# zoltanmaric/h264-fer

Hardware: AMD Instinct MI355X
Metric: macroblocks/sec encode (1080p full-search ME) + bit-exact bitstream vs ref (higher is better)
Workload: dtype u8; 1 GPU; 1080p IPPP encode, full-search +-16 ME (BASELINE configs[2]); content=textured, coded_size=1920x1072, streams_per_gpu=256, contexts_per_gpu=1, gop=30, qp=12, window=32, maxdiff=3, parallelism=1 x 256 independent closed-GOP streams

## Files before the change

h264-fer_amd/csrc/fer_api.hip:

```cpp
#include "fer_ctx.h"
#include "fer_pic_host.h"
#include <stdlib.h>
#include <string.h>

static const int k_qpc[52] = {0,  1,  2,  3,  4,  5,  6,  7,  8,  9,  10, 11, 12, 13, 14, 15, 16, 17,
                              18, 19, 20, 21, 22, 23, 24, 25, 26, 27, 28, 29, 29, 30, 31, 32, 32, 33,
                              34, 34, 35, 35, 36, 36, 37, 37, 37, 38, 38, 38, 39, 39, 39, 39};

extern "C" int ferhip_chroma_qp(int qpy) { return k_qpc[qpy < 0 ? 0 : (qpy > 51 ? 51 : qpy)]; }

int PinnedRing::create(size_t bytes_per_slot, size_t second_bytes)
{
    slot_bytes = bytes_per_slot + second_bytes;
    second_off = bytes_per_slot;
    if (!mem) CK(hipHostMalloc((void **)&mem, slot_bytes * FER_HDR_SLOTS));
    for (int i = 0; i < FER_HDR_SLOTS; i++)
        if (!ev[i]) CK(hipEventCreateWithFlags(&ev[i], hipEventDisableTiming));
    return 0;
}
void *PinnedRing::next()
{
    slot = (slot + 1) % FER_HDR_SLOTS;
    if (hipEventSynchronize(ev[slot]) != hipSuccess) return nullptr;
    return mem + (size_t)slot * slot_bytes;
// ... 1074 lines not shown
    {
        ProfScope ps(c, FERHIP_PH_ME_PRE, 1);
        fer_launch_me_pre(c->d, c->st);
    }
    {
        ProfScope ps(c, FERHIP_PH_ME_WALK, 1);
        fer_launch_me_walk(c->d, c->st);
    }
    if (c->d.speculate) {
        ProfScope ps(c, FERHIP_PH_ME_SPEC, 1);
        fer_launch_me_spec(c->d, c->st);
    }
    {
        ProfScope ps(c, FERHIP_PH_ME_RESOLVE, 1);
        c->d.serial = c->d.serial % 0x7ffffff0 + 1;
        fer_launch_me_resolve(c->d, c->st);
    }
    fer_launch_basic_stat(c->d, c->st);
    fer_launch_p_resid(c->d, c->st);
    CK(hipStreamSynchronize(c->st));
    CK(hipGetLastError());
    return 0;
}

extern "C" size_t ferhip_read_buffer(ferhip_ctx *c, int which, void *dst, size_t cap)
{
    if (!c || !dst) return 0;
    (void)hipSetDevice(c->device);
    if (ctx_sync(c) != hipSuccess) return 0;
    FerDev &d = c->d;
    size_t nm = (size_t)d.nmb * d.S;
    const void *src = nullptr;
    size_t n = 0;
    switch (which) {
    case FERHIP_BUF_INTERP: {
        n = d.ysz * 16 * d.S;
        if (n > cap) return 0;
        for (int pl = 0; pl < 16 * d.S; pl++)
            if (hipMemcpy2D((uint8_t *)dst + (size_t)pl * d.ysz, (size_t)d.W, d.interp + (size_t)pl * d.iplane + d.ioff, (size_t)d.ipitch,
                            (size_t)d.W, (size_t)d.H, hipMemcpyDeviceToHost) != hipSuccess)
                return 0;
        return n;
    }
    case FERHIP_BUF_FEAT: {
        n = d.ysz * 96 * d.S * 2;
        if (n > cap) return 0;
        if (dalloc(c, &d.feat, d.ysz * 96 * d.S)) return 0;
        if (hipDeviceSynchronize() != hipSuccess) return 0;
        fer_launch_features(d, c->st);
        src = d.feat;
        break;
    }
    case FERHIP_BUF_SORTPOS: src = d.sort_pos; n = d.ysz * d.S * 4; break;
    case FERHIP_BUF_KOLIKO: {
        n = (size_t)16385 * d.S * 4;
        if (n > cap) return 0;
        if (hipStreamSynchronize(c->st) != hipSuccess) return 0;
        for (int s = 0; s < d.S; s++) {
            int *o = (int *)dst + (size_t)s * 16385;
            if (hipMemcpy2D(o, 4, d.kol2 + (size_t)s * 16384 * d.kt, (size_t)d.kt * 4, 4, 16385, hipMemcpyDeviceToHost) != hipSuccess)
                return 0;
            for (int a = 0; a <= 16384; a++) o[a] -= (int)((size_t)s * d.ysz);
        }
        return n;
    }
    case FERHIP_BUF_MBTYPE: src = d.mb_type; n = nm * 4; break;
    case FERHIP_BUF_MV: src = d.mv; n = nm * 16; break;
    case FERHIP_BUF_MVD: src = d.mvd; n = nm * 16; break;
    case FERHIP_BUF_LEVELS: src = d.levels; n = nm * FER_LEVELS * 2; break;
    case FERHIP_BUF_CBP: src = d.cbp; n = nm * 2; break;
    case FERHIP_BUF_TC: src = d.tc; n = nm * 24; break;
    case FERHIP_BUF_I4MODE: src = d.i4mode; n = nm * 16; break;
    case FERHIP_BUF_TIMING: src = d.timing; n = 64 * 8; break;
    case FERHIP_BUF_ST2N: src = d.st2n; n = nm * 16; break;
    case FERHIP_BUF_SUMA: src = d.suma; n = nm * 4 * 5 * 4; break;
    case FERHIP_BUF_ST3: src = d.st3; n = nm * 4 * 33 * 3 * 4; break;
    case FERHIP_BUF_ST3N: src = d.st3n; n = nm * 16; break;
    case FERHIP_BUF_V0: src = d.v0; n = nm * 16; break;
    case FERHIP_BUF_SPEC_HDR: src = d.spec_hdr; n = nm * 4 * 16; break;
    case FERHIP_BUF_SPEC_L1: src = d.spec_l1; n = nm * 4 * 17 * 8; break;
    case FERHIP_BUF_SPEC_L2: src = d.spec_l2; n = nm * 4 * 33 * 8; break;
    case FERHIP_BUF_ST2: src = d.st2; n = nm * 4 * FER_ST2_CAP * 8; break;
    case FERHIP_BUF_SPEC_STAT: src = d.spec_stat; n = 8 * 8; break;
    case FERHIP_BUF_MBSIZE: src = d.mbsize; n = nm * 8; break;
    case FERHIP_BUF_CUR:
    case FERHIP_BUF_REF: {
        n = d.ysz * 3 / 2 * d.S;
        if (n > cap) return 0;
        uint8_t *set = c->planes[which == FERHIP_BUF_CUR ? c->cur_set : c->cur_set ^ 1];
        if (copy_frames(c, set, nullptr, (uint8_t *)dst, hipMemcpyDeviceToHost)) return 0;
        if (hipStreamSynchronize(c->st) != hipSuccess) return 0;
        return n;
    }
    default: return 0;
    }
    if (n > cap) return 0;
    if (hipStreamSynchronize(c->st) != hipSuccess) return 0;
    if (hipMemcpy(dst, src, n, hipMemcpyDeviceToHost) != hipSuccess) return 0;
    return n;
}
```

h264-fer_amd/csrc/fer_internal.h:

```cpp
#pragma once
#include "fer_dev.h"
#include "../../include/ferhip.h"

struct FerSortTmp {
    uint4 *rec1;
    uint16_t *keyT;
    uint8_t *dig2;
    uint16_t *skey;
    uint32_t *rec_tmp;
    void *tmp;
    size_t tmp_bytes;
};

size_t fer_sort_tmp_bytes(int n, int S);
void fer_launch_refprep(const FerDev &d, FerSortTmp &t, const int *types, hipStream_t st);
void fer_launch_interp(const FerDev &d, hipStream_t st);
void fer_launch_features(const FerDev &d, hipStream_t st);
void fer_launch_sort(const FerDev &d, FerSortTmp &t, hipStream_t st);
void fer_launch_sort_keys(const FerDev &d, FerSortTmp &t, hipStream_t st);
void fer_launch_sort_radix(const FerDev &d, FerSortTmp &t, hipStream_t st);
void fer_launch_sort_finish(const FerDev &d, FerSortTmp &t, hipStream_t st);
void fer_launch_me_walk(const FerDev &d, hipStream_t st);
void fer_launch_frame_sad(const FerDev &d, const uint8_t *skip, hipStream_t st);
void fer_launch_me_pre(const FerDev &d, hipStream_t st);
void fer_launch_me_spec(const FerDev &d, hipStream_t st);
void fer_launch_me_resolve(const FerDev &d, hipStream_t st);
void fer_launch_basic_stat(const FerDev &d, hipStream_t st);
void fer_launch_p_resid(const FerDev &d, hipStream_t st);
void fer_launch_intra(const FerDev &d, hipStream_t st);
void fer_launch_cavlc(const FerDev &d, hipStream_t st);
void fer_launch_rc_plan(const FerDev &d, hipStream_t st);
int fer_quality_groups(const FerDev &d);
void fer_launch_quality(const FerDev &d, int flags, int slot, hipStream_t st);
void fer_launch_carry_ref(const FerDev &d, hipStream_t st);
void fer_launch_reset_stream(const FerDev &d, int s, int qpw, hipStream_t st);
struct DecLuts;
const DecLuts *dec_luts(hipStream_t st);
void fer_launch_decode_parse(const FerDev &d, const DecBatch &B, hipStream_t st);
void fer_launch_decode_recon(const FerDev &dslice, bool anyP, bool anyIntra, hipStream_t st);
void fer_launch_decode_out(const FerDev &d, const uint8_t *set, const int2 *map, int n, uint8_t *dst, hipStream_t st);
void fer_launch_pad_ingest(const FerDev &d, uint8_t *set, const uint8_t *src, int dw, int dh, const uint8_t *present, hipStream_t st);
void fer_launch_pic_ingest(const FerDev &d, uint8_t *set, const ferhip_pic *d_pics, int format, int dw, int dh, hipStream_t st);
void fer_launch_pic_emit(const FerDev &d, const uint8_t *set, const ferhip_pic *d_pics, int format, const int *win, hipStream_t st);
void fer_launch_pic_emit_slots(const FerDev &d, const uint8_t *set, const int2 *map, int n, uint8_t *dst, int format, uint32_t pitch_y,
                               uint32_t pitch_c, size_t slot_bytes, const int *win, hipStream_t st);
void fer_launch_pic_ingest_packed(const FerDev &d, uint8_t *set, const ferhip_pic *d_pics, int format, int csc, int dw, int dh, hipStream_t st);
void fer_launch_pic_emit_packed(const FerDev &d, const uint8_t *set, const ferhip_pic *d_pics, const int2 *map, int n, uint8_t *dst, int format,
                                int csc, uint32_t pitch, size_t slot_bytes, const int *win, hipStream_t st);
```

h264-fer_amd/csrc/fer_refprep.hip:

```cpp
#include <cstring>
#include <string.h>
#include <algorithm>
#include "fer_internal.h"

#ifndef IT_W
#define IT_W 128
#define IT_H 8
#endif
typedef short s16x2_t __attribute__((ext_vector_type(2)));
#define IT_PITCH (IT_W + 8)
__global__ __launch_bounds__(256) void k_interp(FerDev d)
{
    __shared__ __attribute__((aligned(16))) uint8_t tile[IT_H + 5][IT_PITCH];
    const int s = blockIdx.y;
    if (d.hdr[s * 4 + 3] != 0) return;
    const int W = d.W, H = d.H;
    const uint8_t *R = d.refY + (size_t)s * d.ysz;
    uint8_t *P = d.interp + (size_t)s * 16 * d.iplane + d.ioff;
    const int tw = (W + IT_W - 1) / IT_W;
    const int t = (int)xcd_swizzle(blockIdx.x, gridDim.x);
    const int x0 = (t % tw) * IT_W, y0 = (t / tw) * IT_H;
    const int tid = threadIdx.x;
    {
        constexpr int NL = ((IT_H + 5) * (IT_PITCH / 4) + 255) / 256;
// ... 203 lines not shown
    int nzero = 0;
#pragma unroll
    for (int j = 0; j < 16 + 7; j++) {
        const int r = g * 16 + j;
        const uint32_t *w = (const uint32_t *)&tile[r][x & ~3];
        const uint32_t lo = __builtin_amdgcn_alignbyte(w[1], w[0], (uint32_t)sh);
        const uint32_t hi = __builtin_amdgcn_alignbyte(w[2], w[1], (uint32_t)sh);
        const int a4 = (int)__builtin_amdgcn_sad_u8(lo, 0u, 0u);
        h4[j & 7] = a4;
        h8[j & 7] = (int)__builtin_amdgcn_sad_u8(hi, 0u, (uint32_t)a4);
        hc[j & 7] = (int)__builtin_amdgcn_sad_u8(hi & 0xffffu, 0u, __builtin_amdgcn_sad_u8(lo & 0xffffu, 0u, 0u));
        if (j >= 7) {
            const int yo = r - 7;
            int k0 = 0, k2 = 0, k4 = 0;
#pragma unroll
            for (int k = 0; k < 8; k++) {
                k0 += h8[k];
                k2 += h4[k];
                k4 += hc[k];
            }
            const int k1 = h8[(j + 1) & 7] + h8[(j + 2) & 7] + h8[(j + 3) & 7] + h8[(j + 4) & 7];
            const int k3 = h8[(j + 1) & 7] + h8[(j + 2) & 7] + h8[(j + 5) & 7] + h8[(j + 6) & 7];
            const uint32_t a = (uint32_t)k0 | ((uint32_t)k1 << 16), b = (uint32_t)k2 | ((uint32_t)k3 << 16), c = (uint32_t)k4;
            stage[x][yo] = (uint16_t)k0;
            const int gx = x0 + x, gy = y0 + yo;
            if (gx < W && gy < H) {
                uint32_t *o = (uint32_t *)(d.feat0 + ((size_t)s * d.ysz + (size_t)gy * W + gx) * 6);
                o[0] = a;
                o[1] = b;
                o[2] = c;
                nzero += k0 == 0;
            }
        }
    }
    if (__any(nzero)) {
        const int tot = wave_sum(nzero);
        if ((tid & 63) == 0 && tot) atomicAdd(&d.zero_cnt[s], tot);
    }
    __syncthreads();
    for (int i = tid; i < F0_T * F0_T / 2; i += 256) {
        const int cx = i >> 5, cy = (i & 31) * 2;
        const int gx = x0 + cx, gy = y0 + cy;
        if (gx < W && gy < H)
            *(uint32_t *)(keyT + (size_t)s * d.ysz + (size_t)gx * H + gy) = (uint32_t)stage[cx][cy] | ((uint32_t)stage[cx][cy + 1] << 16);
    }
}

#ifndef RS_THREADS
#define RS_THREADS 512
#endif
#ifndef RS_ITEMS
#define RS_ITEMS 8
#endif
#define RS_TILE (RS_THREADS * RS_ITEMS)
#define RS_BITS 7
#define RS_ND (1 << RS_BITS)

__global__ __launch_bounds__(RS_THREADS) void k_rs_hist(FerDev d, const uint16_t *keyT, const uint8_t *dig2, uint32_t *hist, int ntiles,
                                                       int pass)
{
    __shared__ unsigned h[RS_ND];
    const int s = blockIdx.y, tile = blockIdx.x, tid = threadIdx.x;
    if (d.hdr[s * 4 + 3] != 0) return;
    const int n = d.W * d.H;
    const size_t g0 = (size_t)s * n;
    if (tid < RS_ND) h[tid] = 0;
    static_assert(RS_ITEMS == 8, "one 16-byte / 8-byte load per thread");
    const int idx = tile * RS_TILE + tid * RS_ITEMS;
    const bool ok = idx < n;
    unsigned dgs[RS_ITEMS];
    if (pass == 0) {
        const uint4 v = ok ? *(const uint4 *)(keyT + g0 + idx) : make_uint4(0, 0, 0, 0);
        const uint32_t w[4] = {v.x, v.y, v.z, v.w};
#pragma unroll
        for (int i = 0; i < RS_ITEMS; i++) dgs[i] = (w[i >> 1] >> (16 * (i & 1))) & (RS_ND - 1);
    } else {
        const uint2 v = ok ? *(const uint2 *)(dig2 + g0 + idx) : make_uint2(0, 0);
        const uint32_t w[2] = {v.x, v.y};
#pragma unroll
        for (int i = 0; i < RS_ITEMS; i++) dgs[i] = (w[i >> 2] >> (8 * (i & 3))) & 0xffu;
    }
    __syncthreads();
#pragma unroll
    for (int i = 0; i < RS_ITEMS; i++) {
        const unsigned dg = dgs[i];
        const unsigned d0 = (unsigned)__builtin_amdgcn_readfirstlane((int)dg);
        const unsigned long long same = __ballot(ok && dg == d0);
        if (same && (tid & 63) == __ffsll((long long)same) - 1) atomicAdd(&h[d0], (unsigned)__popcll(same));
        if (ok && dg != d0) atomicAdd(&h[dg], 1u);
    }
    __syncthreads();
    if (tid < RS_ND) hist[((size_t)s * RS_ND + tid) * ntiles + tile] = h[tid];
}

#define RSS_WAVES 16
__global__ __launch_bounds__(64 * RSS_WAVES) void k_rs_scan(FerDev d, uint32_t *hist, int ntiles)
{
    __shared__ unsigned wtot[RSS_WAVES];
    const int s = blockIdx.x, tid = threadIdx.x, lane = tid & 63, wv = tid >> 6;
    if (d.hdr[s * 4 + 3] != 0) return;
    uint4 *h4 = (uint4 *)(hist + (size_t)s * RS_ND * ntiles);
    const int n4 = RS_ND * ntiles / 4;
    const int per = (n4 + RSS_WAVES - 1) / RSS_WAVES;
    const int u0 = min(wv * per, n4), u1 = min(u0 + per, n4);
    unsigned sum = 0;
    for (int u = u0 + lane; u < u1; u += 64) {
        const uint4 v = h4[u];
        sum += v.x + v.y + v.z + v.w;
    }
    sum = (unsigned)wave_sum((int)sum);
    if (lane == 0) wtot[wv] = sum;
    __syncthreads();
    unsigned carry = 0;
    for (int w = 0; w < wv; w++) carry += wtot[w];
    for (int ub = u0; ub < u1; ub += 64) {
        const int u = ub + lane;
        const uint4 v = u < u1 ? h4[u] : make_uint4(0, 0, 0, 0);
        const unsigned t = v.x + v.y + v.z + v.w;
        unsigned inc = t;
#pragma unroll
        for (int o = 1; o < 64; o <<= 1) {
            const unsigned x = __shfl_up(inc, o);
            if (lane >= o) inc += x;
        }
        const unsigned ex = carry + inc - t;
        if (u < u1) h4[u] = make_uint4(ex, ex + v.x, ex + v.x + v.y, ex + v.x + v.y + v.z);
        carry += __shfl(inc, 63);
    }
}

#define RS_SEG_PITCH 12
__device__ __forceinline__ void rs_divmod(unsigned v, unsigned dv, float rdv, unsigned &qo, unsigned &rem)
{
    int q = (int)((float)v * rdv);
    int r = (int)v - q * (int)dv;
    if (r < 0) {
        q--;
        r += (int)dv;
    }
    if (r >= (int)dv) {
        q++;
        r -= (int)dv;
    }
    qo = (unsigned)q;
    rem = (unsigned)r;
}

template <int PASS>
__global__ __launch_bounds__(RS_THREADS) void k_rs_scatter(FerDev d, const uint8_t *dig2_in, const uint4 *rec_in, uint4 *rec1_out,
                                                          uint8_t *dig2_out, uint32_t *rec_tmp, uint16_t *skey, const uint32_t *hist,
                                                          int ntiles)
{
    __shared__ unsigned run[RS_THREADS / 64][RS_ND];
    __shared__ unsigned base[RS_ND], dstart[RS_ND];
    __shared__ unsigned wsum[RS_THREADS / 64];
    __shared__ unsigned long long wtot[RS_THREADS / 64];
    __shared__ __attribute__((aligned(16))) uint4 srec[RS_TILE];
    const int s = blockIdx.y, tile = blockIdx.x, tid = threadIdx.x;
    if (d.hdr[s * 4 + 3] != 0) return;
    const int lane = tid & 63, wv = tid >> 6;
    const int n = d.W * d.H;
    const size_t g0 = (size_t)s * n;
    if (tid < RS_ND) {
#pragma unroll
        for (int w = 0; w < RS_THREADS / 64; w++) run[w][tid] = 0;
        base[tid] = hist[((size_t)s * RS_ND + tid) * ntiles + tile];
    }
    const int w0 = tile * RS_TILE + wv * (RS_TILE / (RS_THREADS / 64));
    unsigned dg[RS_ITEMS], rk[RS_ITEMS];
    uint4 rec[PASS == 0 ? RS_ITEMS : 1];
    if (PASS == 0) {
        const int W = d.W, H = d.H;
        const uint8_t *R = d.refY + (size_t)s * d.ysz;
        uint8_t *smp = (uint8_t *)srec;
        unsigned long long *PL = (unsigned long long *)srec;
        const int t0 = tile * RS_TILE, cnt = min(RS_TILE, n - t0);
        const int xa = t0 / H, ya = t0 - xa * H, xb = (t0 + cnt - 1) / H;
        const int nc = xb - xa + 1, Q = cnt + 7 * nc;
        const int HR = H + 7;
        const float rHR = 1.0f / (float)HR, rH = 1.0f / (float)H;
        const bool shared_box = nc >= 3;
        const int nd0 = ((xb + 7) >> 2) - (xa >> 2) + 1;
        const int nd = shared_box ? (((nd0 | 1) * 4 * HR <= (int)sizeof(srec)) ? (nd0 | 1) : nd0) : RS_SEG_PITCH / 4;
        const int pitch = nd * 4;
        const int rows0 = shared_box ? HR : (nc == 1 ? cnt + 7 : HR - ya);
        {
            const int nboxes = shared_box ? 1 : nc;
            for (int bx = 0; bx < nboxes; bx++) {
                const int nr = bx == 0 ? rows0 : (t0 + cnt - xb * H) + 7;
                const int xs = (xa + bx) & ~3, r0 = (shared_box || bx) ? 0 : ya;
                uint8_t *dst = smp + (bx ? rows0 * RS_SEG_PITCH : 0);
                if (nd <= 7) {
                    const bool inside = xs + nd * 4 <= W;
                    for (int ra = tid; ra < nr; ra += 2 * RS_THREADS) {
                        uint32_t v[2][7];
#pragma unroll
                        for (int k = 0; k < 2; k++) {
                            const int r = ra + k * RS_THREADS;
                            const uint8_t *row = R + (size_t)min(r0 + min(r, nr - 1), H - 1) * W;
                            const uint32_t last = inside ? 0u : (uint32_t)row[W - 1] * 0x01010101u;
#pragma unroll
                            for (int j = 0; j < 7; j++)
                                if (j < nd) v[k][j] = (inside || xs + j * 4 < W) ? *(const uint32_t *)(row + xs + j * 4) : last;
                        }
#pragma unroll
                        for (int k = 0; k < 2; k++) {
                            const int r = ra + k * RS_THREADS;
                            if (r < nr) {
#pragma unroll
                                for (int j = 0; j < 7; j++)
                                    if (j < nd) *(uint32_t *)(dst + r * pitch + j * 4) = v[k][j];
                            }
                        }
                    }
                } else {
                    const float rnd = 1.0f / (float)nd;
                    for (int i0 = 0; i0 < nr * nd; i0 += 8 * RS_THREADS) {
                        uint32_t v[8];
                        int at[8];
#pragma unroll
                        for (int k = 0; k < 8; k++) {
                            const int i = i0 + k * RS_THREADS + tid;
                            at[k] = -1;
                            if (i < nr * nd) {
                                unsigned r, c4;
                                rs_divmod((unsigned)i, (unsigned)nd, rnd, r, c4);
                                const int gx = xs + (int)c4 * 4, gy = min(r0 + (int)r, H - 1);
                                const uint8_t *row = R + (size_t)gy * W;
                                v[k] = gx < W ? *(const uint32_t *)(row + gx) : (uint32_t)row[W - 1] * 0x01010101u;
                                at[k] = (int)r * pitch + (int)c4 * 4;
                            }
                        }
#pragma unroll
                        for (int k = 0; k < 8; k++)
                            if (at[k] >= 0) *(uint32_t *)(dst + at[k]) = v[k];
                    }
                }
            }
        }
        __syncthreads();
        const int L = ((Q + RS_THREADS - 1) / RS_THREADS) | 1;
        const int q0 = min(tid * L, Q), q1 = min(q0 + L, Q);
        unsigned long long hv[13];
        unsigned long long tot = 0;
        {
            unsigned c, r;
            rs_divmod((unsigned)(q0 + ya), (unsigned)HR, rHR, c, r);
#pragma unroll
            for (int k = 0; k < 13; k++) {
                hv[k] = 0;
                if (q0 + k < q1) {
                    int a;
                    if (shared_box)
                        a = (int)r * pitch + (xa & 3) + (int)c;
                    else
                        a = (c ? rows0 * RS_SEG_PITCH + (int)r * RS_SEG_PITCH : ((int)r - ya) * RS_SEG_PITCH) + ((xa + (int)c) & 3);
                    const uint32_t *w = (const uint32_t *)(smp + (a & ~3));
                    const uint32_t sh = (uint32_t)(a & 3);
                    const uint32_t lo = __builtin_amdgcn_alignbyte(w[1], w[0], sh);
                    const uint32_t hi = __builtin_amdgcn_alignbyte(w[2], w[1], sh);
                    const uint32_t a4 = __builtin_amdgcn_sad_u8(lo, 0u, 0u);
                    const uint32_t a8 = __builtin_amdgcn_sad_u8(hi, 0u, a4);
                    const uint32_t ac = __builtin_amdgcn_sad_u8(hi & 0xffffu, 0u, __builtin_amdgcn_sad_u8(lo & 0xffffu, 0u, 0u));
                    hv[k] = ((unsigned long long)ac << 32) | (a8 | (a4 << 16));
                    tot += hv[k];
                    if (++r == (unsigned)HR) {
                        r = 0;
                        c++;
                    }
                }
            }
        }
        unsigned long long inc = tot;
#pragma unroll
        for (int o = 1; o < 64; o <<= 1) {
            const unsigned lo = (unsigned)__shfl_up((int)(unsigned)inc, o), hi = (unsigned)__shfl_up((int)(unsigned)(inc >> 32), o);
            if (lane >= o) inc += ((unsigned long long)hi << 32) | lo;
        }
        if (lane == 63) wtot[wv] = inc;
        __syncthreads();
        unsigned long long pre = inc - tot;
        for (int w = 0; w < wv; w++) pre += wtot[w];
#pragma unroll
        for (int k = 0; k < 13; k++)
            if (q0 + k < q1) {
                PL[q0 + k] = pre;
                pre += hv[k];
            }
        if (q0 < Q && q1 == Q) PL[Q] = pre;
        __syncthreads();
        unsigned x = 0, y = 0;
#pragma unroll
        for (int r = 0; r < RS_ITEMS; r++) {
            const int idx = w0 + r * 64 + lane;
            dg[r] = 0;
            rec[r] = make_uint4(0, 0, 0, 0);
            if (r == 0 || H < 64) {
                rs_divmod((unsigned)min(idx, n - 1), (unsigned)H, rH, x, y);
            } else {
                y += 64;
                if (y >= (unsigned)H) {
                    y -= (unsigned)H;
                    x++;
                }
            }
            if (idx < n) {
                const int c = (int)x - xa;
                const int q = c * HR + (int)y - ya;
                const unsigned long long p0 = PL[q], p8 = PL[q + 8];
                const uint32_t *pl = (const uint32_t *)PL;
                const uint32_t l0 = (uint32_t)p0, l2 = pl[(q + 2) * 2], l4 = pl[(q + 4) * 2], l6 = pl[(q + 6) * 2];
                const unsigned long long dd = p8 - p0;
                const uint32_t k0 = (uint32_t)dd & 0xffffu, k2 = (uint32_t)(dd >> 16) & 0xffffu, k4 = (uint32_t)(dd >> 32) & 0xffffu;
                const uint32_t k1 = (l4 - l0) & 0xffffu, k3 = ((l2 - l0) + (l6 - l4)) & 0xffffu;
                rec[r] = make_uint4(k0 | (k1 << 16), k2 | (k3 << 16), k4, (x << 16) | y);
                dg[r] = k0 & (RS_ND - 1);
            }
        }
    } else {
#pragma unroll
        for (int r = 0; r < RS_ITEMS; r++) {
            const int idx = w0 + r * 64 + lane;
            dg[r] = idx < n ? (unsigned)dig2_in[g0 + idx] : 0u;
        }
    }
    __syncthreads();
    const unsigned long long lt = (1ull << lane) - 1ull;
#pragma unroll
    for (int r = 0; r < RS_ITEMS; r++) {
        const bool ok = w0 + r * 64 + lane < n;
        unsigned long long peers;
        {
            uint32_t dlo = 0, dhi = 0;
#pragma unroll
            for (int b = 0; b < RS_BITS; b++) {
                const unsigned long long bal = __ballot((dg[r] >> b) & 1);
                const uint32_t mine = 0u - ((dg[r] >> b) & 1u);
                dlo |= (uint32_t)bal ^ mine;
                dhi |= (uint32_t)(bal >> 32) ^ mine;
            }
            peers = __ballot(ok) & ~(((unsigned long long)dhi << 32) | dlo);
        }
        const unsigned before = run[wv][dg[r]];
        rk[r] = before + (unsigned)__popcll(peers & lt);
        __builtin_amdgcn_fence(__ATOMIC_SEQ_CST, "wavefront");
        __builtin_amdgcn_wave_barrier();
        if (ok && (peers & lt) == 0) run[wv][dg[r]] = before + (unsigned)__popcll(peers);
        __builtin_amdgcn_fence(__ATOMIC_SEQ_CST, "wavefront");
        __builtin_amdgcn_wave_barrier();
    }
    __syncthreads();
    unsigned tot = 0;
    if (tid < RS_ND) {
#pragma unroll
        for (int w = 0; w < RS_THREADS / 64; w++) {
            unsigned c = run[w][tid];
            run[w][tid] = tot;
            tot += c;
        }
    }
    {
        unsigned inc = tot;
#pragma unroll
        for (int o = 1; o < 64; o <<= 1) {
            unsigned v = __shfl_up(inc, o);
            if (lane >= o) inc += v;
        }
        if (lane == 63) wsum[wv] = inc;
        __syncthreads();
        unsigned before = 0;
        for (int w = 0; w < wv; w++) before += wsum[w];
        if (tid < RS_ND) dstart[tid] = before + inc - tot;
    }
    __syncthreads();
#pragma unroll
    for (int r = 0; r < RS_ITEMS; r++) {
        const int idx = w0 + r * 64 + lane;
        if (idx < n) srec[dstart[dg[r]] + run[wv][dg[r]] + rk[r]] = PASS == 0 ? rec[r] : rec_in[g0 + idx];
    }
    __syncthreads();
    const int cnt = min(RS_TILE, n - tile * RS_TILE);
    if (PASS == 0) {
        for (int i = tid; i < cnt; i += RS_THREADS) {
            const uint4 v = srec[i];
            const unsigned key = v.x & 0xffffu;
            const unsigned dgi = key & (RS_ND - 1);
            const size_t pos = g0 + min(base[dgi] + ((unsigned)i - dstart[dgi]), (unsigned)n - 1u);
            rec1_out[pos] = v;
            dig2_out[pos] = (uint8_t)(key >> RS_BITS);
        }
    } else {
        uint32_t *recs = d.zero_cnt[s] > 0 ? rec_tmp : d.sort_rec;
        for (int i = tid; i < cnt; i += RS_THREADS) {
            const uint4 v = srec[i];
            const unsigned key = v.x & 0xffffu;
            const unsigned dgi = key >> RS_BITS;
            const size_t pos = g0 + base[dgi] + ((unsigned)i - dstart[dgi]);
            uint32_t *o = recs + pos * 3;
            o[0] = v.w;
            o[1] = (v.x >> 16) | (v.y << 16);
            o[2] = (v.y >> 16) | (v.z << 16);
            d.sort_pos[pos] = v.w;
            skey[pos] = (uint16_t)key;
        }
    }
}

#define SI_ITEMS 4
__global__ __launch_bounds__(256) void k_sort_index(FerDev d, const uint16_t *skey)
{
    const int s = blockIdx.y;
    if (d.hdr[s * 4 + 3] != 0) return;
    const int n = d.W * d.H;
    const int nb = 16384 * d.kt;
    uint32_t *kol2 = d.kol2 + (size_t)s * nb;
    const size_t g0 = (size_t)s * n;
    const int lane = threadIdx.x & 63;
    int key[SI_ITEMS], pkey[SI_ITEMS], fkey[SI_ITEMS];
    uint32_t pos[SI_ITEMS], ppos[SI_ITEMS];
#pragma unroll
    for (int k = 0; k < SI_ITEMS; k++) {
        const int i = (blockIdx.x * SI_ITEMS + k) * 256 + (int)threadIdx.x;
        key[k] = pkey[k] = fkey[k] = -1;
        pos[k] = ppos[k] = 0;
        if (i < n) {
            key[k] = (int)skey[g0 + i];
            pos[k] = d.sort_pos[g0 + i];
            if (lane == 0 && i > 0) {
                pkey[k] = (int)skey[g0 + i - 1];
                ppos[k] = d.sort_pos[g0 + i - 1];
            }
            if (i + FER_BRANGE_MIN < n) fkey[k] = (int)skey[g0 + i + FER_BRANGE_MIN];
        }
    }
#pragma unroll
    for (int k = 0; k < SI_ITEMS; k++) {
        const int i = (blockIdx.x * SI_ITEMS + k) * 256 + (int)threadIdx.x;
        int gap_lo = 0, gap_hi = 0;
        uint32_t gval = 0;
        const int nkey = __shfl_up(key[k], 1);
        const uint32_t npos = (uint32_t)__shfl_up((int)pos[k], 1);
        if (i < n) {
            const int pk = lane ? nkey : pkey[k];
            const uint32_t pp = lane ? npos : ppos[k];
            const int bin = key[k] * d.kt + (int)((pos[k] >> 16) >> d.ktw_shift);
            const int prev = i > 0 ? pk * d.kt + (int)((pp >> 16) >> d.ktw_shift) : -1;
            gap_lo = prev + 1;
            gap_hi = bin + 1;
            gval = (uint32_t)(g0 + i);
            if (i == 0 || pk != key[k]) {
                uint4 *br = (uint4 *)(d.brange + ((size_t)s * 16384 + key[k]) * 8);
                br[0] = make_uint4(0, 0, 0, 0);
                br[1] = make_uint4(0, 0, 0, 0);
                *(uint4 *)(d.bmodal + ((size_t)s * 16384 + key[k]) * 4) = make_uint4(0, 0, 0, 0);
            }
// ... 228 lines not shown
```

h264-fer_amd/ferhip.py:

```python
import ctypes as C
import math
import os
from pathlib import Path

import numpy as np

NAL_SLICE, NAL_IDR, NAL_AUTO = 1, 5, 0
NAL_NONE = -1

BUF = dict(INTERP=1, FEAT=2, SORTPOS=3, KOLIKO=4, MBTYPE=5, MV=6, MVD=7, LEVELS=8, CBP=9, TC=10, I4MODE=11,
           CUR=12, REF=13, TIMING=14, ST2N=15, ST2=16, SPEC_STAT=17, MBSIZE=18,
           SUMA=19, ST3=20, ST3N=21, V0=22, SPEC_HDR=23, SPEC_L1=24, SPEC_L2=25)
TUNE_RESOLVE_WGS, TUNE_RESOLVE_GROUP, TUNE_SPECULATE, TUNE_OVERLAP_SORT = 1, 2, 3, 4
RC_CQP, RC_ABR, RC_QUALITY = 0, 1, 2
QM_SSE, QM_SSIM, QUALITY_RING = 1, 2, 64
AU_PARAM_SETS = 1
AU_AVCC = 4
IN_ANNEXB, IN_AVCC = 0, 1
_BUF_DTYPE = {1: np.uint8, 2: np.uint16, 3: np.uint32, 4: np.int32, 5: np.int32, 6: np.int16, 7: np.int16,
              8: np.int16, 9: np.uint8, 10: np.uint8, 11: np.uint8, 12: np.uint8, 13: np.uint8, 14: np.int64, 15: np.int32, 16: np.int32,
              17: np.uint64, 18: np.int32, 19: np.int32, 20: np.int32, 21: np.int32, 22: np.int32, 23: np.int32, 24: np.int32,
              25: np.int32}


class FerHipError(RuntimeError):
    pass


class Params(C.Structure):
    _fields_ = [("qp", C.c_int), ("basic", C.c_int), ("window", C.c_int), ("maxdiff", C.c_int),
                ("intra_every", C.c_int)]


class Rate(C.Structure):
    _fields_ = [("mode", C.c_int), ("qp", C.c_int), ("qp_min", C.c_int), ("qp_max", C.c_int), ("max_step", C.c_int),
                ("ip_offset", C.c_int), ("window", C.c_int), ("target_bits", C.c_longlong), ("target_sse", C.c_longlong)]


class QualityRec(C.Structure):
    _fields_ = [("sse", C.c_uint64 * 3), ("ssim_sum", C.c_double), ("ssim_windows", C.c_uint32), ("qp", C.c_int32),
                ("nal_type", C.c_int32), ("rbsp_bytes", C.c_uint32), ("picture", C.c_uint32)]


_QREC = np.dtype([("sse", np.uint64, 3), ("ssim_sum", np.float64), ("ssim_windows", np.uint32), ("qp", np.int32),
                  ("nal_type", np.int32), ("rbsp_bytes", np.uint32), ("picture", np.uint32)], align=True)
assert _QREC.itemsize == C.sizeof(QualityRec)

AU = np.dtype([("offset", np.uint64), ("bytes", np.uint32), ("nal_type", np.int32)])
NAL_UNIT = np.dtype([("range", np.uint32), ("nal_type", np.int32), ("ref_idc", np.int32), ("bytes", np.uint32), ("offset", np.uint64)])
SPLIT_PREFIX = 64
assert AU.itemsize == 16


class Quality:

    def __init__(self, rec, W, H):
        self.sse = rec["sse"].astype(np.int64)
        n = np.array([W * H, W * H // 4, W * H // 4], np.float64)
        with np.errstate(divide="ignore"):
            self.psnr = 10 * np.log10(255.0 ** 2 * n / self.sse)
        self.ssim_sum = rec["ssim_sum"].copy()
        self.ssim_windows = rec["ssim_windows"].astype(np.int64)
        with np.errstate(divide="ignore", invalid="ignore"):
            self.ssim = np.where(self.ssim_windows > 0, self.ssim_sum / np.maximum(self.ssim_windows, 1), np.nan)
        self.qp = rec["qp"].copy()
        self.nal_type = rec["nal_type"].copy()
        self.rbsp_bytes = rec["rbsp_bytes"].copy()
        self.picture = rec["picture"].copy()


def lib_path():
    return Path(__file__).resolve().parent / "libferhip.so"


_lib = None
# ... 370 lines not shown
        rc = self.lib.ferhip_fetch_nal(self.ctx, int(flags), buf.ctypes.data, int(cap), idx.ctypes.data)
        return rc, buf, idx

    def fetch_nal(self, flags=0, cap=None):
        grow = cap is None
        if grow:
            cap = getattr(self, "_nal_cap", 1 << 20)
        rc, buf, idx = self.fetch_nal_raw(cap, flags)
        if grow and rc == -1 and int(idx["offset"][self.S]) > cap:
            cap = self._nal_cap = 2 * int(idx["offset"][self.S])
            rc, buf, idx = self.fetch_nal_raw(cap, flags)
        _chk(rc, "ferhip_fetch_nal")
        return ([bytes(buf[int(idx["offset"][s]): int(idx["offset"][s]) + int(idx["bytes"][s])]) for s in range(self.S)],
                [int(t) for t in idx["nal_type"][: self.S]])

    def set_rate(self, stream=-1, mode=RC_CQP, qp=None, qp_min=0, qp_max=51, max_step=2, ip_offset=3, window=0,
                 target_bits=0, target_sse=0, target_psnr=None):
        if target_psnr is not None:
            target_sse = self.sse_of_psnr(target_psnr)
        r = Rate(mode, self.params.qp if qp is None else qp, qp_min, qp_max, max_step, ip_offset, window, int(target_bits),
                 int(target_sse))
        _chk(self.lib.ferhip_set_rate(self.ctx, stream, C.byref(r)), "ferhip_set_rate")

    def sse_of_psnr(self, db):
        return int(math.floor(255 ** 2 * self.W * self.H / 10 ** (db / 10)))

    def set_quality(self, flags):
        _chk(self.lib.ferhip_set_quality(self.ctx, int(flags)), "ferhip_set_quality")

    def quality(self, npic=1):
        out = np.zeros((max(int(npic), 1), self.S), _QREC)
        n = self.lib.ferhip_get_quality(self.ctx, int(npic), out.ctypes.data)
        if n < 0:
            raise FerHipError(f"ferhip_get_quality failed with code {n}")
        return Quality(out[:n], self.W, self.H)

    def last_qp(self):
        a = (C.c_int * self.S)()
        _chk(self.lib.ferhip_get_qp(self.ctx, a), "ferhip_get_qp")
        return list(a)

    def fill_interpolated(self):
        _chk(self.lib.ferhip_fill_interpolated(self.ctx), "ferhip_fill_interpolated")

    def inter_encoding(self):
        _chk(self.lib.ferhip_inter_encoding(self.ctx), "ferhip_inter_encoding")

    def read(self, name):
        which = BUF[name]
        n = self.nmb * self.S
        px = self.W * self.H * self.S
        count = {1: px * 16, 2: px * 96, 3: px, 4: 16385 * self.S, 5: n, 6: n * 8, 7: n * 8, 8: n * 400, 9: n * 2,
                 10: n * 24, 11: n * 16, 12: self.fsz * self.S, 13: self.fsz * self.S, 14: 64, 15: n * 4, 16: n * 4 * 384 * 2, 17: 8, 18: n * 2,
                 19: n * 20, 20: n * 4 * 99, 21: n * 4, 22: n * 4, 23: n * 16, 24: n * 4 * 34, 25: n * 4 * 66}[which]
        out = np.empty(count, _BUF_DTYPE[which])
        got = self.lib.ferhip_read_buffer(self.ctx, which, out.ctypes.data, out.nbytes)
        if got != out.nbytes:
            raise FerHipError(f"ferhip_read_buffer({name}) returned {got}, expected {out.nbytes}")
        return out

    PHASES = ("interp", "me_pre", "me_resolve", "p_resid", "intra", "cavlc", "frame_sad", "me_spec", "sort", "me_walk",
              "sort_keys", "sort_finish")
    NPHASE = 12

    def tune(self, key, value):
        _chk(self.lib.ferhip_tune(self.ctx, key, value), "ferhip_tune")

    def profile(self, enable=True):
        _chk(self.lib.ferhip_profile(self.ctx, int(enable)), "ferhip_profile")

    def get_profile(self, reset=True):
        ms = (C.c_double * self.NPHASE)()
        ln = (C.c_long * self.NPHASE)()
        _chk(self.lib.ferhip_get_profile(self.ctx, ms, ln, int(reset)), "ferhip_get_profile")
        return {n: (ms[k], ln[k]) for k, n in enumerate(self.PHASES)}

    def stats(self):
        a = (C.c_int * (5 * self.S))()
        _chk(self.lib.ferhip_get_stats(self.ctx, a), "ferhip_get_stats")
        return np.array(a).reshape(self.S, 5)

    def status(self):
        a = (C.c_int * self.S)()
        _chk(self.lib.ferhip_status(self.ctx, a), "ferhip_status")
        return list(a)


def forward_residual(qp, blocks, keep_dc=False):
    lib = load_library()
    a = np.ascontiguousarray(blocks, np.int32).reshape(-1, 16)
    out = np.empty_like(a)
    _chk(lib.ferhip_forward_residual(qp, a.ctypes.data, out.ctypes.data, int(keep_dc), a.shape[0]),
         "ferhip_forward_residual")
    return out


def inverse_residual(qp, blocks, keep_dc=False):
    lib = load_library()
    a = np.ascontiguousarray(blocks, np.int32).reshape(-1, 16)
    out = np.empty_like(a)
    _chk(lib.ferhip_inverse_residual(qp, a.ctypes.data, out.ctypes.data, int(keep_dc), a.shape[0]),
         "ferhip_inverse_residual")
    return out


class MbJob(C.Structure):
    _fields_ = [("op", C.c_int32), ("cls", C.c_int32), ("qp", C.c_int32), ("qpc", C.c_int32), ("reconstruct", C.c_int32), ("blk", C.c_int32),
# ... 475 lines not shown
```

include/ferhip.h:

```cpp
#ifndef FERHIP_H
#define FERHIP_H
#include <stddef.h>
#include <stdint.h>

#ifdef __cplusplus
extern "C" {
#endif

#define FERHIP_E_ARG -1
#define FERHIP_E_HIP -2
#define FERHIP_E_STATE -3
#define FERHIP_E_UNSUP -4
#define FERHIP_E_DEVICE -5

#define FERHIP_NAL_SLICE 1
#define FERHIP_NAL_IDR 5
#define FERHIP_NAL_AUTO 0
#define FERHIP_NAL_NONE -1

typedef struct ferhip_ctx ferhip_ctx;

typedef struct {
    int qp;
    int basic;
// ... 104 lines not shown

int ferhip_get_stats(ferhip_ctx *c, int *counts5_per_stream);
int ferhip_status(ferhip_ctx *c, int *flags_per_stream);
const char *ferhip_version(void);

#define FERHIP_PH_INTERP 0
#define FERHIP_PH_ME_PRE 1
#define FERHIP_PH_ME_RESOLVE 2
#define FERHIP_PH_P_RESID 3
#define FERHIP_PH_INTRA 4
#define FERHIP_PH_CAVLC 5
#define FERHIP_PH_FRAME_SAD 6
#define FERHIP_PH_ME_SPEC 7
#define FERHIP_PH_SORT 8
#define FERHIP_PH_ME_WALK 9
#define FERHIP_PH_SORT_KEYS 10
#define FERHIP_PH_SORT_FINISH 11
#define FERHIP_NPHASE 12
int ferhip_profile(ferhip_ctx *c, int enable);
#define FERHIP_TUNE_RESOLVE_WGS 1
#define FERHIP_TUNE_RESOLVE_GROUP 2
#define FERHIP_TUNE_OVERLAP_SORT 4
#define FERHIP_TUNE_SPECULATE 3
int ferhip_tune(ferhip_ctx *c, int key, int value);
int ferhip_get_profile(ferhip_ctx *c, double *ms, long *launches, int reset);

int ferhip_fill_interpolated(ferhip_ctx *c);
int ferhip_inter_encoding(ferhip_ctx *c);
#define FERHIP_BUF_INTERP 1
#define FERHIP_BUF_FEAT 2
#define FERHIP_BUF_SORTPOS 3
#define FERHIP_BUF_KOLIKO 4
#define FERHIP_BUF_MBTYPE 5
#define FERHIP_BUF_MV 6
#define FERHIP_BUF_MVD 7
#define FERHIP_BUF_LEVELS 8
#define FERHIP_BUF_CBP 9
#define FERHIP_BUF_TC 10
#define FERHIP_BUF_I4MODE 11
#define FERHIP_BUF_CUR 12
#define FERHIP_BUF_REF 13
#define FERHIP_BUF_TIMING 14
#define FERHIP_BUF_ST2N 15
#define FERHIP_BUF_SPEC_STAT 17
#define FERHIP_BUF_MBSIZE 18
#define FERHIP_BUF_ST2 16
#define FERHIP_BUF_SUMA 19
#define FERHIP_BUF_ST3 20
#define FERHIP_BUF_ST3N 21
#define FERHIP_BUF_V0 22
#define FERHIP_BUF_SPEC_HDR 23
#define FERHIP_BUF_SPEC_L1 24
#define FERHIP_BUF_SPEC_L2 25
size_t ferhip_read_buffer(ferhip_ctx *c, int which, void *dst, size_t cap);
int ferhip_set_reference(ferhip_ctx *c, const void *src);

int ferhip_decode_streams(const uint8_t *const *streams, const size_t *lens, int nstreams, uint8_t *out,
                          int max_pictures, int *pictures, int *width, int *height);
int ferhip_decode_release(void);

typedef struct ferhip_dec ferhip_dec;
int ferhip_dec_create(ferhip_dec **out);
int ferhip_dec_nal(ferhip_dec *d, int nal_unit_type, int nal_ref_idc, const uint8_t *rbsp, size_t n, uint8_t *picture,
                   int *got_picture, int *width, int *height);
void ferhip_dec_destroy(ferhip_dec *d);

typedef struct ferhip_decs ferhip_decs;
int ferhip_decs_create(ferhip_decs **out, int nstreams, int width, int height, int max_pictures);
int ferhip_decs_decode(ferhip_decs *d, const uint8_t *const *chunks, const size_t *lens, uint8_t *out, int out_on_device,
                       int *pictures, int *status);
int ferhip_decs_reset_stream(ferhip_decs *d, int s);
int ferhip_decs_get_crop(ferhip_decs *d, int s, int crop[4] );
int ferhip_decs_set_display(ferhip_decs *d, int x0, int y0, int dw, int dh);
int ferhip_decs_set_layout(ferhip_decs *d, int format, uint32_t pitch_y, uint32_t pitch_c);
int ferhip_decs_set_csc(ferhip_decs *d, int matrix);
void ferhip_decs_destroy(ferhip_decs *d);

#define FERHIP_SPLIT_PREFIX 64
typedef struct { uint32_t range; int32_t nal_type, ref_idc; uint32_t bytes; uint64_t offset; } ferhip_nal_unit;
int ferhip_split_nal_blocks(const uint8_t *ranges, size_t stride, const uint32_t *lens, size_t n, int misalign, uint8_t *out,
                            size_t cap, ferhip_nal_unit *units, size_t units_cap, size_t *nunits);
int ferhip_decs_decode_dev(ferhip_decs *d, const uint8_t *const *d_chunks, const size_t *lens, uint8_t *out, int out_on_device,
                           int *pictures, int *status);
int ferhip_decs_timing(ferhip_decs *d, double *t , int reset);

#define FERHIP_IN_ANNEXB 0
#define FERHIP_IN_AVCC 1
int ferhip_decs_set_input(ferhip_decs *d, int format, int length_size);
int ferhip_decs_set_config(ferhip_decs *d, int s, const uint8_t *avcc, size_t n);
int ferhip_split_avcc_blocks(const uint8_t *ranges, size_t stride, const uint32_t *lens, size_t n, int misalign, int length_size,
                             uint8_t *out, size_t cap, ferhip_nal_unit *units, size_t units_cap, size_t *nunits,
                             int32_t *range_fault );

typedef struct ferhip_y4m ferhip_y4m;
int ferhip_y4m_open(ferhip_y4m **out, const char *path, int *in_width, int *in_height, int *coded_width, int *coded_height);
int ferhip_y4m_read(ferhip_y4m *y, unsigned char *dst);
void ferhip_y4m_close(ferhip_y4m *y);
int ferhip_y4m_write_header(void *file, int width, int height);
int ferhip_y4m_write_frame(void *file, const unsigned char *i420, int width, int height, int with_frame_line);

int ferhip_forward_residual(int qP, const int32_t *in, int32_t *out, int keep_dc, size_t nblocks);
int ferhip_inverse_residual(int qP, const int32_t *in, int32_t *out, int keep_dc, size_t nblocks);
int ferhip_forward_dc_luma_intra(int qP, const int32_t *in, int32_t *out, size_t nblocks);
int ferhip_inverse_dc_luma_intra(int qP, const int32_t *in, int32_t *out, size_t nblocks);
int ferhip_forward_dc_chroma(int qP, const int32_t *in, int32_t *out, size_t nblocks);
int ferhip_inverse_dc_chroma(int qP, const int32_t *in, int32_t *out, size_t nblocks);
// ... 53 lines not shown
```

Before: 22.34 million macroblocks/s.

## Pack radix-sort records into three dwords and shrink scatter LDS footprint

The intermediate sort record between radix passes is bit-packed from a 16-byte uint4 into a 12-byte struct (14-bit key, 13-bit sub-keys, split position bits). This cuts global traffic for rec1 and the shared staging tile. The per-wave run counters become 16-bit, and the scatter kernel gets a waves-per-EU attribute so the smaller LDS use can raise occupancy. The shared-box sample layout is also reworked to fit the smaller region. The cost is extra pack and unpack ALU work, and the tighter bit budgets are guarded by static_asserts. A SORTREC debug read-back buffer is added as well.

```diff
diff --git a/h264-fer_amd/csrc/fer_api.hip b/h264-fer_amd/csrc/fer_api.hip
--- a/h264-fer_amd/csrc/fer_api.hip
+++ b/h264-fer_amd/csrc/fer_api.hip
@@ -1150,6 +1150,7 @@
         break;
     }
     case FERHIP_BUF_SORTPOS: src = d.sort_pos; n = d.ysz * d.S * 4; break;
+    case FERHIP_BUF_SORTREC: src = d.sort_rec; n = d.ysz * d.S * 12; break;
     case FERHIP_BUF_KOLIKO: {
         n = (size_t)16385 * d.S * 4;
         if (n > cap) return 0;
diff --git a/h264-fer_amd/csrc/fer_internal.h b/h264-fer_amd/csrc/fer_internal.h
--- a/h264-fer_amd/csrc/fer_internal.h
+++ b/h264-fer_amd/csrc/fer_internal.h
@@ -1,9 +1,10 @@
 #pragma once
 #include "fer_dev.h"
+#include "fer_sortrec.h"
 #include "../../include/ferhip.h"
 
 struct FerSortTmp {
-    uint4 *rec1;
+    FerSortRec *rec1;
     uint16_t *keyT;
     uint8_t *dig2;
     uint16_t *skey;
diff --git a/h264-fer_amd/csrc/fer_refprep.hip b/h264-fer_amd/csrc/fer_refprep.hip
--- a/h264-fer_amd/csrc/fer_refprep.hip
+++ b/h264-fer_amd/csrc/fer_refprep.hip
@@ -279,9 +279,13 @@
 #ifndef RS_ITEMS
 #define RS_ITEMS 8
 #endif
+#ifndef RS_WAVES_EU
+#define RS_WAVES_EU 6
+#endif
 #define RS_TILE (RS_THREADS * RS_ITEMS)
 #define RS_BITS 7
 #define RS_ND (1 << RS_BITS)
+static_assert(RS_TILE % 256 == 0 && RS_THREADS % 64 == 0 && RS_THREADS >= 2 * 64 && RS_THREADS / 64 * 64 * RS_ITEMS == RS_TILE, "tile shape");
 
 __global__ __launch_bounds__(RS_THREADS) void k_rs_hist(FerDev d, const uint16_t *keyT, const uint8_t *dig2, uint32_t *hist, int ntiles,
                                                        int pass)
@@ -357,6 +361,18 @@
 }
 
 #define RS_SEG_PITCH 12
+#define RS_REGION_BYTES (12 * (RS_TILE + 7 * 3))
+constexpr bool rs_shared_box_fits()
+{
+    for (int nc = 4; nc <= RS_TILE / 16; nc++)
+        if (4 * ((nc + 13) / 4) * ((RS_TILE - 2) / (nc - 2) + 7) > RS_REGION_BYTES) return false;
+    return true;
+}
+static_assert(rs_shared_box_fits(), "a tile of four or more columns keeps its samples in one box");
+static_assert(8 * (RS_TILE + 7 * (RS_TILE / 16) + 1) <= RS_REGION_BYTES, "prefix table PL");
+static_assert(RS_TILE / 48 + 2 <= RS_TILE / 16, "segments of a tile");
+static_assert(sizeof(FerSortRec) == 12 && RS_TILE * sizeof(FerSortRec) <= RS_REGION_BYTES, "staging");
+static_assert(RS_TILE < 65536, "16-bit digit counts and offsets inside a tile");
 __device__ __forceinline__ void rs_divmod(unsigned v, unsigned dv, float rdv, unsigned &qo, unsigned &rem)
 {
     int q = (int)((float)v * rdv);
@@ -374,15 +390,16 @@
 }
 
 template <int PASS>
-__global__ __launch_bounds__(RS_THREADS) void k_rs_scatter(FerDev d, const uint8_t *dig2_in, const uint4 *rec_in, uint4 *rec1_out,
-                                                          uint8_t *dig2_out, uint32_t *rec_tmp, uint16_t *skey, const uint32_t *hist,
-                                                          int ntiles)
-{
-    __shared__ unsigned run[RS_THREADS / 64][RS_ND];
+__global__ __launch_bounds__(RS_THREADS) __attribute__((amdgpu_waves_per_eu(RS_WAVES_EU, RS_WAVES_EU))) void k_rs_scatter(
+    FerDev d, const uint8_t *dig2_in, const FerSortRec *rec_in, FerSortRec *rec1_out, uint8_t *dig2_out, uint32_t *rec_tmp, uint16_t *skey,
+    const uint32_t *hist, int ntiles)
+{
+    __shared__ uint16_t run[RS_THREADS / 64][RS_ND];
     __shared__ unsigned base[RS_ND], dstart[RS_ND];
     __shared__ unsigned wsum[RS_THREADS / 64];
     __shared__ unsigned long long wtot[RS_THREADS / 64];
-    __shared__ __attribute__((aligned(16))) uint4 srec[RS_TILE];
+    __shared__ __attribute__((aligned(16))) uint32_t sreg[RS_REGION_BYTES / 4];
+    FerSortRec *srec = (FerSortRec *)sreg;
     const int s = blockIdx.y, tile = blockIdx.x, tid = threadIdx.x;
     if (d.hdr[s * 4 + 3] != 0) return;
     const int lane = tid & 63, wv = tid >> 6;
@@ -395,28 +412,28 @@
     }
     const int w0 = tile * RS_TILE + wv * (RS_TILE / (RS_THREADS / 64));
     unsigned dg[RS_ITEMS], rk[RS_ITEMS];
-    uint4 rec[PASS == 0 ? RS_ITEMS : 1];
+    FerSortRec rec[PASS == 0 ? RS_ITEMS : 1];
     if (PASS == 0) {
         const int W = d.W, H = d.H;
         const uint8_t *R = d.refY + (size_t)s * d.ysz;
-        uint8_t *smp = (uint8_t *)srec;
-        unsigned long long *PL = (unsigned long long *)srec;
+        uint8_t *smp = (uint8_t *)sreg;
+        unsigned long long *PL = (unsigned long long *)sreg;
         const int t0 = tile * RS_TILE, cnt = min(RS_TILE, n - t0);
         const int xa = t0 / H, ya = t0 - xa * H, xb = (t0 + cnt - 1) / H;
         const int nc = xb - xa + 1, Q = cnt + 7 * nc;
         const int HR = H + 7;
         const float rHR = 1.0f / (float)HR, rH = 1.0f / (float)H;
-        const bool shared_box = nc >= 3;
         const int nd0 = ((xb + 7) >> 2) - (xa >> 2) + 1;
-        const int nd = shared_box ? (((nd0 | 1) * 4 * HR <= (int)sizeof(srec)) ? (nd0 | 1) : nd0) : RS_SEG_PITCH / 4;
+        const bool shared_box = nc >= 3 && nd0 * 4 * HR <= RS_REGION_BYTES;
+        const int nd = shared_box ? (((nd0 | 1) * 4 * HR <= RS_REGION_BYTES) ? (nd0 | 1) : nd0) : RS_SEG_PITCH / 4;
         const int pitch = nd * 4;
         const int rows0 = shared_box ? HR : (nc == 1 ? cnt + 7 : HR - ya);
         {
             const int nboxes = shared_box ? 1 : nc;
             for (int bx = 0; bx < nboxes; bx++) {
-                const int nr = bx == 0 ? rows0 : (t0 + cnt - xb * H) + 7;
+                const int nr = bx == 0 ? rows0 : (bx == nc - 1 ? (t0 + cnt - xb * H) + 7 : HR);
                 const int xs = (xa + bx) & ~3, r0 = (shared_box || bx) ? 0 : ya;
-                uint8_t *dst = smp + (bx ? rows0 * RS_SEG_PITCH : 0);
+                uint8_t *dst = smp + (bx ? (bx * HR - ya) * RS_SEG_PITCH : 0);
                 if (nd <= 7) {
                     const bool inside = xs + nd * 4 <= W;
                     for (int ra = tid; ra < nr; ra += 2 * RS_THREADS) {
@@ -481,7 +498,7 @@
                     if (shared_box)
                         a = (int)r * pitch + (xa & 3) + (int)c;
                     else
-                        a = (c ? rows0 * RS_SEG_PITCH + (int)r * RS_SEG_PITCH : ((int)r - ya) * RS_SEG_PITCH) + ((xa + (int)c) & 3);
+                        a = (q0 + k) * RS_SEG_PITCH + ((xa + (int)c) & 3);
                     const uint32_t *w = (const uint32_t *)(smp + (a & ~3));
                     const uint32_t sh = (uint32_t)(a & 3);
                     const uint32_t lo = __builtin_amdgcn_alignbyte(w[1], w[0], sh);
@@ -521,7 +538,7 @@
         for (int r = 0; r < RS_ITEMS; r++) {
             const int idx = w0 + r * 64 + lane;
             dg[r] = 0;
-            rec[r] = make_uint4(0, 0, 0, 0);
+            rec[r] = FerSortRec{0, 0, 0};
             if (r == 0 || H < 64) {
                 rs_divmod((unsigned)min(idx, n - 1), (unsigned)H, rH, x, y);
             } else {
@@ -540,7 +557,7 @@
                 const unsigned long long dd = p8 - p0;
                 const uint32_t k0 = (uint32_t)dd & 0xffffu, k2 = (uint32_t)(dd >> 16) & 0xffffu, k4 = (uint32_t)(dd >> 32) & 0xffffu;
                 const uint32_t k1 = (l4 - l0) & 0xffffu, k3 = ((l2 - l0) + (l6 - l4)) & 0xffffu;
-                rec[r] = make_uint4(k0 | (k1 << 16), k2 | (k3 << 16), k4, (x << 16) | y);
+                rec[r] = fer_sortrec_pack(k0, k1, k2, k3, k4, x, y);
                 dg[r] = k0 & (RS_ND - 1);
             }
         }
@@ -572,7 +589,7 @@
         rk[r] = before + (unsigned)__popcll(peers & lt);
         __builtin_amdgcn_fence(__ATOMIC_SEQ_CST, "wavefront");
         __builtin_amdgcn_wave_barrier();
-        if (ok && (peers & lt) == 0) run[wv][dg[r]] = before + (unsigned)__popcll(peers);
+        if (ok && (peers & lt) == 0) run[wv][dg[r]] = (uint16_t)(before + (unsigned)__popcll(peers));
         __builtin_amdgcn_fence(__ATOMIC_SEQ_CST, "wavefront");
         __builtin_amdgcn_wave_barrier();
     }
@@ -582,7 +599,7 @@
 #pragma unroll
         for (int w = 0; w < RS_THREADS / 64; w++) {
             unsigned c = run[w][tid];
-            run[w][tid] = tot;
+            run[w][tid] = (uint16_t)tot;
             tot += c;
         }
     }
@@ -609,8 +626,8 @@
     const int cnt = min(RS_TILE, n - tile * RS_TILE);
     if (PASS == 0) {
         for (int i = tid; i < cnt; i += RS_THREADS) {
-            const uint4 v = srec[i];
-            const unsigned key = v.x & 0xffffu;
+            const FerSortRec v = srec[i];
+            const unsigned key = v.a & ((1u << FER_SR_K0_BITS) - 1u);
             const unsigned dgi = key & (RS_ND - 1);
             const size_t pos = g0 + min(base[dgi] + ((unsigned)i - dstart[dgi]), (unsigned)n - 1u);
             rec1_out[pos] = v;
@@ -619,15 +636,15 @@
     } else {
         uint32_t *recs = d.zero_cnt[s] > 0 ? rec_tmp : d.sort_rec;
         for (int i = tid; i < cnt; i += RS_THREADS) {
-            const uint4 v = srec[i];
-            const unsigned key = v.x & 0xffffu;
+            uint32_t key, txy, k12, k34;
+            fer_sortrec_unpack(srec[i], key, txy, k12, k34);
             const unsigned dgi = key >> RS_BITS;
             const size_t pos = g0 + base[dgi] + ((unsigned)i - dstart[dgi]);
             uint32_t *o = recs + pos * 3;
-            o[0] = v.w;
-            o[1] = (v.x >> 16) | (v.y << 16);
-            o[2] = (v.y >> 16) | (v.z << 16);
-            d.sort_pos[pos] = v.w;
+            o[0] = txy;
+            o[1] = k12;
+            o[2] = k34;
+            d.sort_pos[pos] = txy;
             skey[pos] = (uint16_t)key;
         }
     }
diff --git a/h264-fer_amd/csrc/fer_sortrec.h b/h264-fer_amd/csrc/fer_sortrec.h
--- /dev/null
+++ b/h264-fer_amd/csrc/fer_sortrec.h
@@ -0,0 +1,40 @@
+#pragma once
+#include <stdint.h>
+#if defined(__HIPCC__)
+#define FER_SR_FN __host__ __device__ __forceinline__
+#else
+#define FER_SR_FN inline
+#endif
+
+#define FER_SR_K0_BITS 14
+#define FER_SR_KN_BITS 13
+#define FER_SR_POS_BITS 14
+static_assert(64 * 255 < (1 << FER_SR_K0_BITS) && 32 * 255 < (1 << FER_SR_KN_BITS) && 16384 <= (1 << FER_SR_POS_BITS), "field ranges");
+static_assert(FER_SR_K0_BITS + 4 * FER_SR_KN_BITS + 2 * FER_SR_POS_BITS <= 96, "the record is three dwords");
+static_assert(FER_SR_K0_BITS + FER_SR_KN_BITS + 5 == 32 && 2 * FER_SR_KN_BITS + 6 == 32 && FER_SR_KN_BITS + FER_SR_POS_BITS + 3 <= 32 &&
+                  5 + 6 + 3 == FER_SR_POS_BITS,
+              "dword budgets");
+
+struct FerSortRec {
+    uint32_t a;
+    uint32_t b;
+    uint32_t c;
+};
+
+FER_SR_FN FerSortRec fer_sortrec_pack(uint32_t k0, uint32_t k1, uint32_t k2, uint32_t k3, uint32_t k4, uint32_t tx, uint32_t ty)
+{
+    FerSortRec r;
+    r.a = k0 | (k1 << 14) | ((ty & 31u) << 27);
+    r.b = k2 | (k3 << 13) | (((ty >> 5) & 63u) << 26);
+    r.c = k4 | (tx << 13) | ((ty >> 11) << 27);
+    return r;
+}
+
+FER_SR_FN void fer_sortrec_unpack(const FerSortRec &r, uint32_t &k0, uint32_t &pos, uint32_t &k12, uint32_t &k34)
+{
+    k0 = r.a & 0x3fffu;
+    const uint32_t ty = (r.a >> 27) | ((r.b >> 26) << 5) | ((r.c >> 27) << 11);
+    pos = (((r.c >> 13) & 0x3fffu) << 16) | ty;
+    k12 = ((r.a >> 14) & 0x1fffu) | ((r.b & 0x1fffu) << 16);
+    k34 = ((r.b >> 13) & 0x1fffu) | ((r.c & 0x1fffu) << 16);
+}
diff --git a/h264-fer_amd/ferhip.py b/h264-fer_amd/ferhip.py
--- a/h264-fer_amd/ferhip.py
+++ b/h264-fer_amd/ferhip.py
@@ -10,7 +10,7 @@
 
 BUF = dict(INTERP=1, FEAT=2, SORTPOS=3, KOLIKO=4, MBTYPE=5, MV=6, MVD=7, LEVELS=8, CBP=9, TC=10, I4MODE=11,
            CUR=12, REF=13, TIMING=14, ST2N=15, ST2=16, SPEC_STAT=17, MBSIZE=18,
-           SUMA=19, ST3=20, ST3N=21, V0=22, SPEC_HDR=23, SPEC_L1=24, SPEC_L2=25)
+           SUMA=19, ST3=20, ST3N=21, V0=22, SPEC_HDR=23, SPEC_L1=24, SPEC_L2=25, SORTREC=26)
 TUNE_RESOLVE_WGS, TUNE_RESOLVE_GROUP, TUNE_SPECULATE, TUNE_OVERLAP_SORT = 1, 2, 3, 4
 RC_CQP, RC_ABR, RC_QUALITY = 0, 1, 2
 QM_SSE, QM_SSIM, QUALITY_RING = 1, 2, 64
@@ -20,7 +20,7 @@
 _BUF_DTYPE = {1: np.uint8, 2: np.uint16, 3: np.uint32, 4: np.int32, 5: np.int32, 6: np.int16, 7: np.int16,
               8: np.int16, 9: np.uint8, 10: np.uint8, 11: np.uint8, 12: np.uint8, 13: np.uint8, 14: np.int64, 15: np.int32, 16: np.int32,
               17: np.uint64, 18: np.int32, 19: np.int32, 20: np.int32, 21: np.int32, 22: np.int32, 23: np.int32, 24: np.int32,
-              25: np.int32}
+              25: np.int32, 26: np.uint32}
 
 
 class FerHipError(RuntimeError):
@@ -497,7 +497,7 @@
         px = self.W * self.H * self.S
         count = {1: px * 16, 2: px * 96, 3: px, 4: 16385 * self.S, 5: n, 6: n * 8, 7: n * 8, 8: n * 400, 9: n * 2,
                  10: n * 24, 11: n * 16, 12: self.fsz * self.S, 13: self.fsz * self.S, 14: 64, 15: n * 4, 16: n * 4 * 384 * 2, 17: 8, 18: n * 2,
-                 19: n * 20, 20: n * 4 * 99, 21: n * 4, 22: n * 4, 23: n * 16, 24: n * 4 * 34, 25: n * 4 * 66}[which]
+                 19: n * 20, 20: n * 4 * 99, 21: n * 4, 22: n * 4, 23: n * 16, 24: n * 4 * 34, 25: n * 4 * 66, 26: px * 3}[which]
         out = np.empty(count, _BUF_DTYPE[which])
         got = self.lib.ferhip_read_buffer(self.ctx, which, out.ctypes.data, out.nbytes)
         if got != out.nbytes:
diff --git a/include/ferhip.h b/include/ferhip.h
--- a/include/ferhip.h
+++ b/include/ferhip.h
@@ -180,6 +180,7 @@
 #define FERHIP_BUF_SPEC_HDR 23
 #define FERHIP_BUF_SPEC_L1 24
 #define FERHIP_BUF_SPEC_L2 25
+#define FERHIP_BUF_SORTREC 26
 size_t ferhip_read_buffer(ferhip_ctx *c, int which, void *dst, size_t cap);
 int ferhip_set_reference(ferhip_ctx *c, const void *src);
 
```

Result: faster. 22.65 million macroblocks/s (median of 6 runs) (+1.4%).
